# JoeMWatson/input-inference-for-control

Measured on AMD Instinct MI355X. Metric: i2c timestep-messages/sec (cell-iterations/s = B*T*EM-iters/s), pendulum T=200 B=4096 per GPU, higher is better.
Workload: dtype f64; 1 GPU; pendulum_known_quad cubature i2c (nx=2, nu=1, nz=4), T=200, B=4096 trajectories per GPU, global batch 4096, CubatureQuadrature(1,0,0), alpha0=100, tol=0; batch_per_gpu=4096, horizon=200, parallelism=batch-sharded x1, no collective in the EM loop, kernels=one lane per trajectory

## Files before the change

input-inference-for-control_amd/csrc/i2c_cell.hpp:

```cpp
#pragma once
#include <stdint.h>
#include <type_traits>
#include "../../include/i2c_hip.h"
#include "i2c_linalg.hpp"
#include "i2c_models.hpp"

namespace i2c {

template <typename R> struct Rule {
  R sf;
  R w0;
  R wi;
  R W;
  int unit;
  int gh_degree, gh_points;
  R gh_x[I2C_MAX_GH_DEGREE], gh_w[I2C_MAX_GH_DEGREE];
};

template <class M> struct PerTraj : M {};
template <class M> struct is_per_traj : std::false_type {};
template <class M> struct is_per_traj<PerTraj<M>> : std::true_type {};
template <typename R, bool PER_TRAJ> struct ParamsB {};
template <typename R> struct ParamsB<R, true> {
  const R* params_b;
// ... 120 lines not shown
  I2C_HD static constexpr int lin(int) { return -1; }
  I2C_HD static constexpr int dep(int) { return DIN - 1; }
};

template <class M, class ST, int DIN, int DOUT, bool CROSS, bool UNITW = false, typename R, class F>
I2C_FN void sp_transform(const Rule<R>& rule, const R* m, const R* Sin, const R* L, const F& f, R* my, R* Sy,
                         R* Sxy, const PolyTab<R>* tab = nullptr) {
  constexpr int NA = M::NA, NA1 = NA > 0 ? NA : 1;
  R s0[NA1], c0[NA1];
#pragma unroll
  for (int a = 0; a < NA; ++a) {
    if (tab)
      r_sincos(m[M::ang(a)], *tab, &s0[a], &c0[a]);
    else
      r_sincos(m[M::ang(a)], &s0[a], &c0[a]);
  }
  R y0[DOUT];
  f(m, s0, c0, y0);
  R A[DOUT];
#pragma unroll
  for (int k = 0; k < DOUT; ++k) A[k] = R(0);
#pragma unroll
  for (int k = 0; k < sym(DOUT); ++k) Sy[k] = R(0);
  if (CROSS) {
#pragma unroll
    for (int k = 0; k < DIN * DOUT; ++k) Sxy[k] = R(0);
  }
#pragma unroll
  for (int j = 0; j < DIN; ++j) {
    bool any = false;
#pragma unroll
    for (int k = 0; k < DOUT; ++k) any = any || (ST::lin(k) < 0 && ST::dep(k) >= j);
    R a[DOUT], dl[DOUT];
    if (any) {
      R xp[DIN], xm[DIN];
#pragma unroll
      for (int i = 0; i < DIN; ++i) {
        if (i < j) {
          xp[i] = m[i];
          xm[i] = m[i];
        } else {
          const R d = rule.sf * L[tri(i, j)];
          xp[i] = m[i] + d;
          xm[i] = m[i] - d;
        }
      }
      R sp[NA1], cp[NA1], sm[NA1], cm[NA1];
#pragma unroll
      for (int q = 0; q < NA; ++q) {
        if (M::ang(q) < j) {
          sp[q] = sm[q] = s0[q];
          cp[q] = cm[q] = c0[q];
        } else {
          R sd, cd;
          if (tab)
            r_sincos(rule.sf * L[tri(M::ang(q), j)], *tab, &sd, &cd);
          else
            r_sincos_small(rule.sf * L[tri(M::ang(q), j)], &sd, &cd);
          sp[q] = s0[q] * cd + c0[q] * sd;
          cp[q] = c0[q] * cd - s0[q] * sd;
          sm[q] = s0[q] * cd - c0[q] * sd;
          cm[q] = c0[q] * cd + s0[q] * sd;
        }
      }
      R yp[DOUT], ym[DOUT];
      f(xp, sp, cp, yp);
      f(xm, sm, cm, ym);
#pragma unroll
      for (int k = 0; k < DOUT; ++k) {
        a[k] = (yp[k] - y0[k]) + (ym[k] - y0[k]);
        dl[k] = yp[k] - ym[k];
      }
    }
#pragma unroll
    for (int k = 0; k < DOUT; ++k) {
      const bool nl_k = ST::lin(k) < 0 && ST::dep(k) >= j;
      if (ST::lin(k) >= j) dl[k] = R(2) * rule.sf * L[tri(ST::lin(k) >= j ? ST::lin(k) : j, j)];
      if (nl_k) A[k] += a[k];
#pragma unroll
      for (int l = 0; l <= k; ++l) {
        const bool nl_l = ST::lin(l) < 0 && ST::dep(l) >= j;
        const bool d_k = nl_k || ST::lin(k) >= j, d_l = nl_l || ST::lin(l) >= j;
        const bool both_lin = ST::lin(k) >= 0 && ST::lin(l) >= 0;
        if (nl_k && nl_l) Sy[tri(k, l)] += a[k] * a[l];
        if (d_k && d_l && !both_lin) Sy[tri(k, l)] += dl[k] * dl[l];
      }
      if (CROSS && nl_k) {
#pragma unroll
        for (int i = j; i < DIN; ++i) Sxy[i * DOUT + k] += L[tri(i, j)] * dl[k];
      }
    }
    sched_fence<(DIN >= 6)>();
  }
  const R hw = R(0.5) * rule.wi, w2 = rule.wi * rule.wi, cs = rule.wi * rule.sf;
#pragma unroll
  for (int k = 0; k < DOUT; ++k) {
    const R Wk = UNITW ? R(1) : rule.W;
    my[k] = ST::lin(k) >= 0 ? Wk * m[ST::lin(k) >= 0 ? ST::lin(k) : 0] : Wk * y0[k] + rule.wi * A[k];
#pragma unroll
    for (int l = 0; l <= k; ++l) {
      if (ST::lin(k) >= 0 && ST::lin(l) >= 0)
        Sy[tri(k, l)] = Sin[tri_any(ST::lin(k) >= 0 ? ST::lin(k) : 0, ST::lin(l) >= 0 ? ST::lin(l) : 0)];
      else
        Sy[tri(k, l)] = hw * Sy[tri(k, l)] - w2 * A[k] * A[l];
    }
    if (CROSS) {
#pragma unroll
      for (int i = 0; i < DIN; ++i)
        Sxy[i * DOUT + k] = ST::lin(k) >= 0 ? Sin[tri_any(i, ST::lin(k) >= 0 ? ST::lin(k) : 0)] : cs * Sxy[i * DOUT + k];
    }
  }
  if (!UNITW && !rule.unit) {
    const R omw = R(1) - rule.W;
    R yc[DOUT];
#pragma unroll
    for (int k = 0; k < DOUT; ++k) yc[k] = ST::lin(k) >= 0 ? m[ST::lin(k) >= 0 ? ST::lin(k) : 0] : y0[k];
#pragma unroll
    for (int k = 0; k < DOUT; ++k)
#pragma unroll
      for (int l = 0; l <= k; ++l)
        Sy[tri(k, l)] += omw * (rule.W * yc[k] * yc[l] + rule.wi * (A[k] * yc[l] + yc[k] * A[l]));
  }
}

template <int DX, int DZ, typename R>
I2C_FN bool kalman_update(R* mu, R* S, const R* mz, R* Sz, R* Sxz, const R* zt) {
  R rinv[DZ];
  const bool ok = chol<DZ>(Sz, rinv);
  R q[DZ];
#pragma unroll
  for (int k = 0; k < DZ; ++k) q[k] = zt[k] - mz[k];
  fsub<DZ>(Sz, rinv, q);
#pragma unroll
  for (int i = 0; i < DX; ++i) {
    fsub<DZ>(Sz, rinv, &Sxz[i * DZ]);
    R v = mu[i];
#pragma unroll
    for (int k = 0; k < DZ; ++k) v += Sxz[i * DZ + k] * q[k];
    mu[i] = v;
    sched_fence<(DZ >= 8)>();
  }
#pragma unroll
  for (int i = 0; i < DX; ++i)
#pragma unroll
    for (int j = 0; j <= i; ++j) {
      R v = S[tri(i, j)];
#pragma unroll
      for (int k = 0; k < DZ; ++k) v -= Sxz[i * DZ + k] * Sxz[j * DZ + k];
      S[tri(i, j)] = v;
    }
  return ok;
}

template <int N, typename R> I2C_FN R pdf_ratio(R* S, const R* delta, bool* ok, const PolyTab<R>* tab = nullptr) {
  R rinv[N], q[N];
  *ok = chol<N>(S, rinv);
#pragma unroll
  for (int i = 0; i < N; ++i) q[i] = delta[i];
  fsub<N>(S, rinv, q);
  R maha = R(0);
#pragma unroll
  for (int i = 0; i < N; ++i) maha += q[i] * q[i];
  (void)tab;
  return r_exp(R(-0.5) * maha);
}

template <int NX, int NU, typename R>
I2C_FN void joint_from_gain(const R* mu_x, const R* sig_x, const R* Kt, const R* qmu_x, const R* qmu_u,
                            const R* sig_u, R* mu0, R* S0) {
  constexpr int D = NX + NU;
#pragma unroll
  for (int i = 0; i < NX; ++i) mu0[i] = mu_x[i];
#pragma unroll
  for (int a = 0; a < NU; ++a) {
    R v = qmu_u[a];
#pragma unroll
    for (int k = 0; k < NX; ++k) v += Kt[a * NX + k] * (mu_x[k] - qmu_x[k]);
    mu0[NX + a] = v;
  }
#pragma unroll
  for (int i = 0; i < NX; ++i)
#pragma unroll
    for (int j = 0; j <= i; ++j) S0[tri(i, j)] = sig_x[tri(i, j)];
#pragma unroll
  for (int a = 0; a < NU; ++a) {
#pragma unroll
    for (int j = 0; j < NX; ++j) {
      R v = R(0);
#pragma unroll
      for (int k = 0; k < NX; ++k) v += Kt[a * NX + k] * sig_x[tri_any(k, j)];
      S0[tri(NX + a, j)] = v;
    }
#pragma unroll
    for (int c = 0; c <= a; ++c) S0[tri(NX + a, NX + c)] = sig_u[tri(a, c)];
  }
  (void)D;
}

template <int NX, int NU, typename R> I2C_FN void gain_quad(const R* Kt, const R* sig, R* out) {
  R KS[NU * NX];
#pragma unroll
  for (int a = 0; a < NU; ++a)
#pragma unroll
    for (int j = 0; j < NX; ++j) {
      R v = R(0);
#pragma unroll
      for (int k = 0; k < NX; ++k) v += Kt[a * NX + k] * sig[tri_any(k, j)];
      KS[a * NX + j] = v;
    }
#pragma unroll
  for (int a = 0; a < NU; ++a)
#pragma unroll
    for (int c = 0; c <= a; ++c) {
      R v = R(0);
#pragma unroll
      for (int j = 0; j < NX; ++j) v += KS[a * NX + j] * Kt[c * NX + j];
      out[tri(a, c)] = v;
    }
}

I2C_FN int note_failure(int fail, bool ok, int reason, int t) {
  return (fail == 0 && !ok) ? ((reason << 16) | (t + 1)) : fail;
}
I2C_FN int flag_stage(int cell_bad, bool ok, int order) {
  const int v = ok ? 0 : 7 - order;
  return cell_bad > v ? cell_bad : v;
}
I2C_FN int fold_cell_failure(int fail, int cell_bad, int t) {
  const int order = 7 - cell_bad;
  const int reason = order == 0 ? 2 : (order == 1 ? 1 : order + 1);
  return (fail == 0 && cell_bad != 0) ? ((reason << 16) | (t + 1)) : fail;
}
I2C_FN void set_status(int32_t* status, int b, int reason, int t) {
  if (status[b] == 0) status[b] = (reason << 16) | (t + 1);
}

template <class M, int DIN, int DOUT, bool CROSS, typename R, class F>
I2C_FN void grid_transform(const Rule<R>& rule, const R* m, const R* L, const F& f, R* my, R* Sy, R* Sxy) {
  constexpr int NA = M::NA, NA1 = NA > 0 ? NA : 1;
  R sn[NA1], cs[NA1], y0[DOUT], s1[DOUT];
#pragma unroll
  for (int a = 0; a < NA; ++a) r_sincos(m[M::ang(a)], &sn[a], &cs[a]);
  f(m, sn, cs, y0);
#pragma unroll
  for (int k = 0; k < DOUT; ++k) s1[k] = R(0);
#pragma unroll
  for (int k = 0; k < sym(DOUT); ++k) Sy[k] = R(0);
  if (CROSS) {
#pragma unroll
    for (int k = 0; k < DIN * DOUT; ++k) Sxy[k] = R(0);
  }
  int dig[DIN];
#pragma unroll
  for (int i = 0; i < DIN; ++i) dig[i] = 0;
  const int deg = rule.gh_degree;
  for (int p = 0; p < rule.gh_points; ++p) {
    R xi[DIN], w = R(1);
#pragma unroll
    for (int i = 0; i < DIN; ++i) {
      R xv = rule.gh_x[0], wv = rule.gh_w[0];
#pragma unroll
      for (int q = 1; q < I2C_MAX_GH_DEGREE; ++q) {
        xv = dig[i] == q ? rule.gh_x[q] : xv;
        wv = dig[i] == q ? rule.gh_w[q] : wv;
      }
      xi[i] = xv;
      w *= wv;
    }
    R dx[DIN], x[DIN], y[DOUT];
#pragma unroll
    for (int i = 0; i < DIN; ++i) {
      R v = R(0);
#pragma unroll
      for (int j = 0; j <= i; ++j) v += L[tri(i, j)] * xi[j];
      dx[i] = rule.sf * v;
      x[i] = m[i] + dx[i];
    }
#pragma unroll
    for (int a = 0; a < NA; ++a) r_sincos(x[M::ang(a)], &sn[a], &cs[a]);
    f(x, sn, cs, y);
#pragma unroll
    for (int k = 0; k < DOUT; ++k) y[k] -= y0[k];
#pragma unroll
    for (int k = 0; k < DOUT; ++k) {
      const R wy = w * y[k];
      s1[k] += wy;
#pragma unroll
      for (int l = 0; l <= k; ++l) Sy[tri(k, l)] += wy * y[l];
      if (CROSS) {
#pragma unroll
        for (int i = 0; i < DIN; ++i) Sxy[i * DOUT + k] += dx[i] * wy;
      }
    }
    bool carry = true;
#pragma unroll
    for (int i = 0; i < DIN; ++i) {
      const int nd = dig[i] + (carry ? 1 : 0);
      carry = nd >= deg;
      dig[i] = carry ? 0 : nd;
    }
  }
#pragma unroll
  for (int k = 0; k < DOUT; ++k) my[k] = y0[k] + s1[k];
#pragma unroll
  for (int k = 0; k < DOUT; ++k)
#pragma unroll
    for (int l = 0; l <= k; ++l) Sy[tri(k, l)] -= s1[k] * s1[l];
}

template <class M, int DEG, int DIN, int DOUT, bool CROSS, typename R, class F>
I2C_FN void grid_transform_ct(const Rule<R>& rule, const R* m, const R* L, const F& f, R* my, R* Sy, R* Sxy) {
  static_assert(DIN >= 1 && DIN <= 3, "unrolled grid: up to three input dimensions");
  constexpr int NA = M::NA, NA1 = NA > 0 ? NA : 1;
  R sn[NA1], cs[NA1], y0[DOUT], s1[DOUT];
#pragma unroll
  for (int a = 0; a < NA; ++a) r_sincos(m[M::ang(a)], &sn[a], &cs[a]);
  f(m, sn, cs, y0);
#pragma unroll
  for (int k = 0; k < DOUT; ++k) s1[k] = R(0);
#pragma unroll
  for (int k = 0; k < sym(DOUT); ++k) Sy[k] = R(0);
  if (CROSS) {
#pragma unroll
    for (int k = 0; k < DIN * DOUT; ++k) Sxy[k] = R(0);
  }
  R xs[DEG], ws[DEG];
#pragma unroll
  for (int q = 0; q < DEG; ++q) xs[q] = rule.sf * rule.gh_x[q], ws[q] = rule.gh_w[q];
  constexpr int N1 = DIN > 1 ? DEG : 1, N2 = DIN > 2 ? DEG : 1;
#pragma unroll
  for (int i0 = 0; i0 < DEG; ++i0) {
    R d0[DIN];
#pragma unroll
    for (int i = 0; i < DIN; ++i) d0[i] = L[tri(i, 0)] * xs[i0];
#pragma unroll
    for (int a = 0; a < NA; ++a)
      if (M::ang(a) == 0) r_sincos(m[0] + d0[0], &sn[a], &cs[a]);
#pragma unroll
    for (int i1 = 0; i1 < N1; ++i1) {
      R d1[DIN];
      R w1 = ws[i0];
#pragma unroll
      for (int i = 0; i < DIN; ++i) d1[i] = d0[i];
      if constexpr (DIN > 1) {
#pragma unroll
        for (int i = 1; i < DIN; ++i) d1[i] += L[tri(i, 1)] * xs[i1];
        w1 *= ws[i1];
#pragma unroll
        for (int a = 0; a < NA; ++a)
          if (M::ang(a) == 1) r_sincos(m[1] + d1[1], &sn[a], &cs[a]);
      }
      R part[DOUT];
#pragma unroll
      for (int k = 0; k < DOUT; ++k) part[k] = R(0);
#pragma unroll
      for (int i2 = 0; i2 < N2; ++i2) {
        R dx[DIN], x[DIN], y[DOUT];
        R w = w1;
#pragma unroll
        for (int i = 0; i < DIN; ++i) dx[i] = d1[i];
        if constexpr (DIN > 2) {
          dx[2] += L[tri(2, 2)] * xs[i2];
          w *= ws[i2];
#pragma unroll
          for (int a = 0; a < NA; ++a)
            if (M::ang(a) == 2) r_sincos(m[2] + dx[2], &sn[a], &cs[a]);
        }
#pragma unroll
        for (int i = 0; i < DIN; ++i) x[i] = m[i] + dx[i];
        f(x, sn, cs, y);
#pragma unroll
        for (int k = 0; k < DOUT; ++k) {
          const R wy = w * (y[k] - y0[k]);
          y[k] -= y0[k];
          part[k] += wy;
#pragma unroll
          for (int l = 0; l <= k; ++l) Sy[tri(k, l)] += wy * y[l];
          if (CROSS) Sxy[(DIN - 1) * DOUT + k] += dx[DIN - 1] * wy;
        }
      }
#pragma unroll
      for (int k = 0; k < DOUT; ++k) {
        s1[k] += part[k];
        if (CROSS) {
#pragma unroll
          for (int i = 0; i < DIN - 1; ++i) Sxy[i * DOUT + k] += d1[i] * part[k];
        }
      }
    }
  }
#pragma unroll
  for (int k = 0; k < DOUT; ++k) my[k] = y0[k] + s1[k];
#pragma unroll
  for (int k = 0; k < DOUT; ++k)
#pragma unroll
    for (int l = 0; l <= k; ++l) Sy[tri(k, l)] -= s1[k] * s1[l];
}

template <bool GRID, class M, class ST, int DIN, int DOUT, bool CROSS, bool UNITW = false, typename R, class F>
I2C_FN void transform(const Rule<R>& rule, const R* m, const R* Sin, const R* L, const F& f, R* my, R* Sy, R* Sxy,
                      const PolyTab<R>* tab = nullptr) {
  if constexpr (GRID) {
    if constexpr (DIN <= 3) {
      if (rule.gh_degree == 3) return grid_transform_ct<M, 3, DIN, DOUT, CROSS>(rule, m, L, f, my, Sy, Sxy);
      if (rule.gh_degree == 4) return grid_transform_ct<M, 4, DIN, DOUT, CROSS>(rule, m, L, f, my, Sy, Sxy);
      if (rule.gh_degree == 2) return grid_transform_ct<M, 2, DIN, DOUT, CROSS>(rule, m, L, f, my, Sy, Sxy);
    }
    grid_transform<M, DIN, DOUT, CROSS>(rule, m, L, f, my, Sy, Sxy);
  } else
    sp_transform<M, ST, DIN, DOUT, CROSS, UNITW>(rule, m, Sin, L, f, my, Sy, Sxy, tab);
}


template <typename R, typename S = R> struct FwdArgs {
  const S* prior;
  S* fwd;
  S* prior_out;
  const R* x0;
  const R* sig_x0;
  const R* z;
  const R* alpha;
  const R* alpha_cell;
  const uint8_t* ff;
  int32_t* status;
  const uint8_t* expert;
};

template <class M, typename R, bool LEAN = false, bool GRID = false, typename ST_ = R>
I2C_HD inline void forward_sweep_body(const Consts<M, R>& c, const FwdArgs<R, ST_>& a, const int b) {
  using C = Consts<M, R>;
  constexpr int NX = C::NX, NU = C::NU, NZ = C::NZ, NZT = C::NZT, D = C::D;
  constexpr unsigned W = sizeof(ST_);
  const unsigned long B = c.B;
  const int T = c.T;
  const unsigned bo = (unsigned)b * W;
  const unsigned rb0 = (unsigned)(B * W);
  const R alpha_traj = a.alpha[b];
  int fail = 0;

  R mu_x[NX], sig_x[sym(NX)];
#pragma unroll
  for (int i = 0; i < NX; ++i) mu_x[i] = a.x0[i * B + b];
#pragma unroll
  for (int i = 0; i < sym(NX); ++i) sig_x[i] = a.sig_x0[i * B + b];

  constexpr bool VOFF = C::D <= 5;
  unsigned voff[VOFF ? C::E_FWD : 1];
  if (VOFF) {
#pragma unroll
    for (int e = 0; e < C::E_FWD; ++e) voff[e] = bo + (unsigned)e * rb0;
  }
  constexpr bool PREFETCH = C::D <= 5;
  R pri[C::E_PRI], zt[NZ];
  if (PREFETCH) {
    const unsigned rb = rb0;
    const Window w = make_window(a.prior + (unsigned long)(LEAN ? 0 : c.row(0)) * C::E_POST * B, (unsigned long)C::E_POST * rb);
#pragma unroll
    for (int e = 0; e < C::E_PRI; ++e) pri[e] = (R)wld<ST_>(w, VOFF ? 0u : (e) * rb, VOFF ? voff[e] : bo);
#pragma unroll
    for (int k = 0; k < NZ; ++k) zt[k] = (!LEAN && c.z_per_cell) ? a.z[((long)c.row(0) * NZ + k) * B + b] : c.zg[k];
  }

  unsigned ff_cur = a.ff[LEAN ? 0 : c.row(0)];
  constexpr bool STRUCT_L0 = C::D <= 5;
  R Lx[STRUCT_L0 ? sym(NX) : 1];
  if (STRUCT_L0) {
    R rx[NX];
#pragma unroll
    for (int i = 0; i < sym(NX); ++i) Lx[i] = sig_x[i];
    fail = note_failure(fail, chol<NX>(Lx, rx), 1, 0);
  }

  ff_cur = opaque(ff_cur);
  if (PREFETCH) {
#pragma unroll
    for (int e = 0; e < C::E_PRI; ++e) pri[e] = opaque(pri[e]);
#pragma unroll
    for (int k = 0; k < NZ; ++k) zt[k] = opaque(zt[k]);
  }
#pragma unroll
  for (int i = 0; i < NX; ++i) mu_x[i] = opaque(mu_x[i]);
#pragma unroll
  for (int i = 0; i < sym(NX); ++i) sig_x[i] = opaque(sig_x[i]);
  const R alpha_settled = opaque(alpha_traj);
  R alpha_cur = opaque((!LEAN && a.alpha_cell) ? a.alpha_cell[(long)c.row(0) * B + b] : alpha_settled);
  constexpr bool CONST_V = VOFF && (sym(NZ) + sym(NX) <= 16);
  PolyTab<R> ptab;
  if (CONST_V) poly_tab_init(ptab);
  const PolyTab<R>* const tab = CONST_V ? &ptab : nullptr;
  R xi0_v[CONST_V ? sym(NZ) : 1], eta_v[CONST_V ? sym(NX) : 1];
  if (CONST_V) {
#pragma unroll
    for (int i = 0; i < sym(NZ); ++i) xi0_v[i] = opaque(c.sig_xi0[i]);
#pragma unroll
    for (int i = 0; i < sym(NX); ++i) eta_v[i] = opaque(LEAN ? c.sig_eta[i] : c.sig_eta_w[i]);
  }

  for (int t = 0; t < T; ++t) {
    const int tn = t + 1 < T ? t + 1 : t;
    const int tr = LEAN ? t : c.row(t), tnr = LEAN ? tn : c.row(tn);
    const unsigned rb = opaque_uniform(rb0);
    const int kz = (C::D >= 6) ? (int)opaque_uniform(0u) : 0;
    if (!PREFETCH) {
      const Window w = make_window(a.prior + (unsigned long)tr * C::E_POST * B, (unsigned long)C::E_POST * rb);
#pragma unroll
      for (int e = 0; e < C::E_PRI; ++e) pri[e] = (R)wld<ST_>(w, VOFF ? 0u : (e) * rb, VOFF ? voff[e] : bo);
#pragma unroll
      for (int k = 0; k < NZ; ++k) zt[k] = (!LEAN && c.z_per_cell) ? a.z[((long)tr * NZ + k) * B + b] : c.zg[k];
    }

    const R alpha = opaque(alpha_cur);
    const R* pmu = pri;
    const R* psig = pri + D;
    const R* Kprev = pri + D + sym(D);

    int cell_bad = 0;
    R mu0[D], S0[sym(D)];
    R L0[STRUCT_L0 ? sym(D) : 1], Luu[sym(NU)], ruu[NU];
    if (ff_cur != 0) {
#pragma unroll
      for (int i = 0; i < NX; ++i) mu0[i] = mu_x[i];
#pragma unroll
      for (int i = NX; i < D; ++i) mu0[i] = pmu[i];
#pragma unroll
      for (int i = 0; i < D; ++i)
#pragma unroll
        for (int j = 0; j <= i; ++j)
          S0[tri(i, j)] = (i < NX) ? sig_x[tri(i, j)] : (j >= NX ? psig[tri(i, j)] : R(0));
      if (STRUCT_L0) {
#pragma unroll
        for (int p = 0; p < NU; ++p)
#pragma unroll
          for (int q = 0; q <= p; ++q) Luu[tri(p, q)] = psig[tri(NX + p, NX + q)];
#pragma unroll
        for (int p = 0; p < NU; ++p)
#pragma unroll
          for (int j = 0; j < NX; ++j) L0[tri(NX + p, j)] = R(0);
      }
    } else {
      R S[sym(NX)], delta[NX];
#pragma unroll
      for (int i = 0; i < sym(NX); ++i) S[i] = psig[i] + sig_x[i];
#pragma unroll
      for (int i = 0; i < NX; ++i) delta[i] = mu_x[i] - pmu[i];
      bool ok;
      const R rho = pdf_ratio<NX>(S, delta, &ok, tab);
      cell_bad = flag_stage(cell_bad, ok, 0);
      R Kt[NU * NX];
#pragma unroll
      for (int i = 0; i < NU * NX; ++i) Kt[i] = rho * Kprev[i];
      R sig_u[sym(NU)];
      gain_quad<NX, NU>(Kt, sig_x, sig_u);
#pragma unroll
      for (int p = 0; p < NU; ++p)
#pragma unroll
        for (int q = 0; q <= p; ++q) {
          R v = psig[tri(NX + p, NX + q)];
#pragma unroll
          for (int k = 0; k < NX; ++k) v -= Kt[p * NX + k] * psig[tri(NX + q, k)];
          Luu[tri(p, q)] = v;
          sig_u[tri(p, q)] += v;
        }
      joint_from_gain<NX, NU>(mu_x, sig_x, Kt, pmu, pmu + NX, sig_u, mu0, S0);
      if (STRUCT_L0) {
#pragma unroll
        for (int p = 0; p < NU; ++p)
#pragma unroll
          for (int j = 0; j < NX; ++j) {
            R v = R(0);
#pragma unroll
            for (int k = j; k < NX; ++k) v += Kt[p * NX + k] * Lx[tri(k, j)];
            L0[tri(NX + p, j)] = v;
          }
      }
    }
    if (STRUCT_L0) {
#pragma unroll
      for (int i = 0; i < sym(NX); ++i) L0[i] = Lx[i];
      cell_bad = flag_stage(cell_bad, chol<NU>(Luu, ruu), 1);
#pragma unroll
      for (int p = 0; p < NU; ++p)
#pragma unroll
        for (int q = 0; q <= p; ++q) L0[tri(NX + p, NX + q)] = Luu[tri(p, q)];
    }
    if (!LEAN && a.prior_out) {
      const Window w = make_window(a.prior_out + (unsigned long)t * (D + sym(D)) * B, (unsigned long)(D + sym(D)) * rb);
#pragma unroll
      for (int e = 0; e < D; ++e) wst(w, VOFF ? 0u : (e) * rb, VOFF ? voff[e] : bo, (ST_)mu0[e]);
#pragma unroll
      for (int e = 0; e < sym(D); ++e) wst(w, VOFF ? 0u : (D + e) * rb, VOFF ? voff[D + e] : bo, (ST_)S0[e]);
    }

    ff_cur = a.ff[tnr];
    if (!LEAN && a.alpha_cell) alpha_cur = a.alpha_cell[(long)tnr * B + b];
    if (PREFETCH) {
      const Window w = make_window(a.prior + (unsigned long)tnr * C::E_POST * B, (unsigned long)C::E_POST * rb);
#pragma unroll
      for (int e = 0; e < C::E_PRI; ++e) pri[e] = (R)wld<ST_>(w, VOFF ? 0u : (e) * rb, VOFF ? voff[e] : bo);
    }

    sched_fence<(D >= 6)>();
    {
      R Lf[STRUCT_L0 ? 1 : sym(D)], rinv[D];
      if (!STRUCT_L0) {
#pragma unroll
        for (int i = 0; i < sym(D); ++i) Lf[i] = S0[i];
        cell_bad = flag_stage(cell_bad, chol<D>(Lf, rinv), 1);
      }
      const R* L = STRUCT_L0 ? L0 : Lf;
      R mz[NZ], Sz[sym(NZ)], Sxz[D * NZ];
      transform<GRID, M, ObsStruct<M>, D, NZ, true, LEAN>(c.rule_xu, mu0, S0, L, ObserveF<M, R>{params_of(c, b)}, mz, Sz, Sxz, tab);
#pragma unroll
      for (int i = 0; i < sym(NZ); ++i) Sz[i] += alpha * (CONST_V ? xi0_v[i] : c.sig_xi0[i + kz]);
      cell_bad = flag_stage(cell_bad, kalman_update<D, NZ>(mu0, S0, mz, Sz, Sxz, zt), 2);
    }
    if (!LEAN && PREFETCH && c.z_per_cell) {
#pragma unroll
      for (int k = 0; k < NZ; ++k) zt[k] = a.z[((long)tnr * NZ + k) * B + b];
    }
    const Window out = make_window(a.fwd + (unsigned long)t * C::E_FWD * B, (unsigned long)C::E_FWD * rb);
#pragma unroll
    for (int e = 0; e < D; ++e) wst(out, VOFF ? 0u : (e) * rb, VOFF ? voff[e] : bo, (ST_)mu0[e]);
#pragma unroll
    for (int e = 0; e < sym(D); ++e) wst(out, VOFF ? 0u : (D + e) * rb, VOFF ? voff[D + e] : bo, (ST_)S0[e]);

    sched_fence<(D >= 6)>();
    R Sxy[D * NX];
    {
      R L[sym(D)], rinv[D];
#pragma unroll
      for (int i = 0; i < sym(D); ++i) L[i] = S0[i];
      cell_bad = flag_stage(cell_bad, chol<D>(L, rinv), 3);
      transform<GRID, M, DenseStruct<D>, D, NX, true, LEAN>(c.rule_xu, mu0, S0, L, DynamicsF<M, R>{params_of(c, b)}, mu_x, sig_x, Sxy, tab);
    }
#pragma unroll
    for (int i = 0; i < sym(NX); ++i) sig_x[i] += CONST_V ? eta_v[i] : (LEAN ? c.sig_eta[i + kz] : c.sig_eta_w[i + kz]);
    R L3[sym(NX)], rinv3[NX];
#pragma unroll
    for (int i = 0; i < sym(NX); ++i) L3[i] = sig_x[i];
    cell_bad = flag_stage(cell_bad, chol<NX>(L3, rinv3), 4);
    sched_fence<(D >= 6)>();
#pragma unroll
    for (int i = 0; i < D; ++i) {
      fsub<NX>(L3, rinv3, &Sxy[i * NX]);
      bsub<NX>(L3, rinv3, &Sxy[i * NX]);
      sched_fence<(D >= 6)>();
    }

    ff_cur = opaque(ff_cur);
    if (!LEAN) {
      alpha_cur = opaque(alpha_cur);
      if (PREFETCH) {
#pragma unroll
        for (int k = 0; k < NZ; ++k) zt[k] = opaque(zt[k]);
      }
    }
    if (PREFETCH) {
#pragma unroll
      for (int e = 0; e < C::E_PRI; ++e) pri[e] = opaque(pri[e]);
    }
#pragma unroll
    for (int e = 0; e < D * NX; ++e) wst(out, VOFF ? 0u : (D + sym(D) + NX + sym(NX) + e) * rb, VOFF ? voff[D + sym(D) + NX + sym(NX) + e] : bo, (ST_)Sxy[e]);
    sched_fence<(D >= 6)>();

    if (NZT > 0 && t == c.terminal_cell && c.has_Qf) {
      constexpr int NT = C::NZT1;
      R mzt[NT], Szt[sym(NT)], Sxzt[NX * NT];
      transform<GRID, M, TermStruct<M>, NX, NT, true, LEAN>(c.rule_x, mu_x, sig_x, L3, ObserveTermF<M, R>{params_of(c, b)}, mzt, Szt, Sxzt);
#pragma unroll
      for (int i = 0; i < sym(NT); ++i) Szt[i] += alpha * c.sig_xiT0[i];
      cell_bad = flag_stage(cell_bad, kalman_update<NX, NT>(mu_x, sig_x, mzt, Szt, Sxzt, c.zg_term), 5);
      if (STRUCT_L0) {
#pragma unroll
        for (int i = 0; i < sym(NX); ++i) L3[i] = sig_x[i];
        cell_bad = flag_stage(cell_bad, chol<NX>(L3, rinv3), 5);
      }
    }
    if (STRUCT_L0) {
#pragma unroll
      for (int i = 0; i < sym(NX); ++i) Lx[i] = L3[i];
    }
    fail = fold_cell_failure(fail, cell_bad, t);
#pragma unroll
    for (int e = 0; e < NX; ++e) wst(out, VOFF ? 0u : (D + sym(D) + e) * rb, VOFF ? voff[D + sym(D) + e] : bo, (ST_)mu_x[e]);
#pragma unroll
    for (int e = 0; e < sym(NX); ++e) wst(out, VOFF ? 0u : (D + sym(D) + NX + e) * rb, VOFF ? voff[D + sym(D) + NX + e] : bo, (ST_)sig_x[e]);

  }
  if (fail != 0 && a.status[b] == 0) a.status[b] = fail;
}


template <class M, typename R>
I2C_FN void end_of_chain(const Consts<M, R>& c, R* temp, const int b, const R* m3f, const R* S3f, R* m3m, R* S3m,
                         int32_t* status) {
  constexpr int NX = M::NX;
  if (c.has_x_terminal) {
    const R tmp = temp[b];
    temp[b] = tmp + c.dtemp;
    R St[sym(NX)], Ssum[sym(NX)], rinv[NX];
#pragma unroll
    for (int i = 0; i < sym(NX); ++i) {
      St[i] = tmp * S3f[i];
      Ssum[i] = c.sig_x_term[i] + St[i];
    }
    bool ok = chol<NX>(Ssum, rinv);
    R Wm[NX * NX];
#pragma unroll
    for (int j = 0; j < NX; ++j) {
      R col[NX];
#pragma unroll
      for (int i = 0; i < NX; ++i) col[i] = St[tri_any(i, j)];
      fsub<NX>(Ssum, rinv, col);
#pragma unroll
      for (int i = 0; i < NX; ++i) Wm[i * NX + j] = col[i];
    }
#pragma unroll
    for (int i = 0; i < NX; ++i)
#pragma unroll
      for (int j = 0; j <= i; ++j) {
        R v = St[tri(i, j)];
#pragma unroll
        for (int k = 0; k < NX; ++k) v -= Wm[k * NX + i] * Wm[k * NX + j];
        S3m[tri(i, j)] = v;
      }
    R r1[NX], r2[NX], Lt[sym(NX)], LT[sym(NX)];
#pragma unroll
    for (int i = 0; i < sym(NX); ++i) {
      Lt[i] = St[i];
      LT[i] = c.sig_x_term[i];
    }
    ok = chol<NX>(Lt, rinv) && ok;
#pragma unroll
    for (int i = 0; i < NX; ++i) r1[i] = m3f[i];
    fsub<NX>(Lt, rinv, r1);
    bsub<NX>(Lt, rinv, r1);
    ok = chol<NX>(LT, rinv) && ok;
#pragma unroll
    for (int i = 0; i < NX; ++i) r2[i] = c.mu_x_term[i];
    fsub<NX>(LT, rinv, r2);
    bsub<NX>(LT, rinv, r2);
#pragma unroll
    for (int i = 0; i < NX; ++i) r1[i] += r2[i];
    symv<NX>(S3m, r1, m3m);
    if (!ok) set_status(status, b, 6, c.T - 1);
  } else {
#pragma unroll
    for (int i = 0; i < NX; ++i) m3m[i] = m3f[i];
#pragma unroll
    for (int i = 0; i < sym(NX); ++i) S3m[i] = S3f[i];
  }
}

template <int N, typename R>
I2C_FN void gaussian_cost(const R* W, const bool w_diag, const R* mz, const R* Sz, const R* zt, R* m, R* v) {
  R err[N];
#pragma unroll
  for (int i = 0; i < N; ++i) err[i] = mz[i] - zt[i];
  if (w_diag) {
    R mm = R(0), tr2 = R(0), quad = R(0), we[N];
#pragma unroll
    for (int i = 0; i < N; ++i) {
      we[i] = W[tri(i, i)] * err[i];
      mm += we[i] * err[i] + W[tri(i, i)] * Sz[tri(i, i)];
    }
#pragma unroll
    for (int i = 0; i < N; ++i)
#pragma unroll
      for (int j = 0; j <= i; ++j) {
        const R sww = Sz[tri(i, j)] * (W[tri(i, i)] * W[tri(j, j)]);
        tr2 += (i == j ? R(1) : R(2)) * Sz[tri(i, j)] * sww;
        quad += (i == j ? R(1) : R(2)) * Sz[tri(i, j)] * (we[i] * we[j]);
      }
    *m = mm;
    *v = R(2) * tr2 + R(4) * quad;
    return;
  }
  R We[N];
  symv<N>(W, err, We);
  R SW[N * N];
#pragma unroll
  for (int i = 0; i < N; ++i)
#pragma unroll
    for (int j = 0; j < N; ++j) {
      R s = R(0);
#pragma unroll
      for (int k = 0; k < N; ++k) s += Sz[tri_any(i, k)] * W[tri_any(k, j)];
      SW[i * N + j] = s;
    }
  R mm = R(0), tr2 = R(0), quad = R(0);
#pragma unroll
  for (int i = 0; i < N; ++i) {
    mm += err[i] * We[i] + SW[i * N + i];
    R SWe = R(0);
#pragma unroll
    for (int j = 0; j < N; ++j) {
      tr2 += SW[i * N + j] * SW[j * N + i];
      SWe += Sz[tri_any(i, j)] * We[j];
    }
    quad += We[i] * SWe;
  }
  *m = mm;
  *v = R(2) * tr2 + R(4) * quad;
}

template <class M, typename R, bool GRID = false>
I2C_FN R terminal_obs_stats(const Consts<M, R>& c, const int b, const R* m3m, const R* S3m, R* term_stats,
                            int32_t* status) {
  using C = Consts<M, R>;
  constexpr int NX = C::NX, NZT = C::NZT;
  const long B = c.B;
  R trT = R(0);
  if (NZT > 0 && c.has_Qf) {
    constexpr int NT = C::NZT1;
    R L3[sym(NX)], rinv3[NX], mzt[NT], Szt[sym(NT)];
#pragma unroll
    for (int i = 0; i < sym(NX); ++i) L3[i] = S3m[i];
    if (!chol<NX>(L3, rinv3)) set_status(status, b, 6, c.T - 1);
    transform<GRID, M, TermStruct<M>, NX, NT, false>(c.rule_x, m3m, S3m, L3, ObserveTermF<M, R>{params_of(c, b)}, mzt, Szt,
                                                  (R*)nullptr);
    R tv;
    gaussian_cost<NT>(c.Qf, c.qf_diag != 0, mzt, Szt, c.zg_term, &trT, &tv);
#pragma unroll
    for (int k = 0; k < NT; ++k) term_stats[(long)(3 + k) * B + b] = mzt[k];
#pragma unroll
    for (int k = 0; k < sym(NT); ++k) term_stats[(long)(3 + NT + k) * B + b] = Szt[k];
  }
  term_stats[b] = trT;
  return trT;
}

template <class M, typename R, bool GRID = false>
I2C_FN bool cell_posterior(const Consts<M, R>& c, const int b, const R* zt, R* mu, R* S, const R* J, const R* dm, const R* dS,
                           R* ctl, R* mz, R* Sz, R* cm, R* cv, const PolyTab<R>* tab = nullptr) {
  using C = Consts<M, R>;
// ... 972 lines not shown
```

input-inference-for-control_amd/csrc/i2c_linalg.hpp:

```cpp
#pragma once

#ifdef I2C_HOST_SIM
#include <cmath>
#define I2C_HD
#else
#include <hip/hip_runtime.h>
#define I2C_HD __host__ __device__
#endif
#define I2C_FN I2C_HD static inline __attribute__((always_inline))

namespace i2c {

constexpr int sym(int n) { return n * (n + 1) / 2; }
constexpr int tri(int i, int j) { return i * (i + 1) / 2 + j; }
constexpr int tri_any(int i, int j) { return i >= j ? tri(i, j) : tri(j, i); }

#ifdef I2C_HOST_SIM
I2C_FN double seed_rsq(double x) { return (double)(float)(1.0 / std::sqrt(x)); }
I2C_FN double seed_rcp(double x) { return (double)(float)(1.0 / x); }
I2C_FN double m_fma(double a, double b, double c) { return std::fma(a, b, c); }
I2C_FN double m_rint(double x) { return std::rint(x); }
I2C_FN double m_fabs(double x) { return std::fabs(x); }
I2C_FN float r_rsqrt(float x) { return 1.0f / std::sqrt(x); }
I2C_FN float r_rcp(float x) { return 1.0f / x; }
I2C_FN double r_exp(double x) { return std::exp(x); }
I2C_FN float r_exp(float x) { return std::exp(x); }
I2C_FN double r_log(double x) { return std::log(x); }
I2C_FN float r_log(float x) { return std::log(x); }
I2C_FN void r_sincos(float x, float* s, float* c) { *s = std::sin(x); *c = std::cos(x); }
#else
I2C_FN double seed_rsq(double x) { return __builtin_amdgcn_rsq(x); }
I2C_FN double seed_rcp(double x) { return __builtin_amdgcn_rcp(x); }
I2C_FN double m_fma(double a, double b, double c) { return fma(a, b, c); }
I2C_FN double m_rint(double x) { return rint(x); }
I2C_FN double m_fabs(double x) { return fabs(x); }
I2C_FN float r_rsqrt(float x) { return rsqrtf(x); }
I2C_FN float r_rcp(float x) { return 1.0f / x; }
I2C_FN float r_exp(float x) { return expf(x); }
I2C_FN double r_log(double x) { return log(x); }
I2C_FN float r_log(float x) { return logf(x); }
I2C_FN void r_sincos(float x, float* s, float* c) { sincosf(x, s, c); }
#endif

#ifdef I2C_HOST_SIM
I2C_FN double p_fma(double p, double z, double c) { return std::fma(p, z, c); }
#else
I2C_FN double p_fma(double p, double z, double c) {
  double r;
  asm("v_fma_f64 %0, %1, %2, %3" : "=v"(r) : "v"(p), "v"(z), "v"(c));
  return r;
}
#endif

I2C_FN double r_rsqrt(double x) {
  const double y = seed_rsq(x);
  const double e = m_fma(-(x * y), y, 1.0);
  return m_fma(y * e, m_fma(e, 0.375, 0.5), y);
}
I2C_FN double r_rcp(double x) {
  double y = seed_rcp(x);
  y = m_fma(m_fma(-x, y, 1.0), y, y);
  return m_fma(m_fma(-x, y, 1.0), y, y);
}
#ifndef I2C_HOST_SIM
I2C_FN double r_exp(double x) {
  const double n = m_rint(x * 1.44269504088896338700e+00);
  double r = m_fma(-n, 6.93147180369123816490e-01, x);
  r = m_fma(-n, 1.90821492927058770002e-10, r);
  const double z = r * r;
  double e = p_fma(2.08767569878681e-09, z, 2.755731922398589e-07);
  double o = p_fma(1.6059043836821613e-10, z, 2.505210838544172e-08);
  e = p_fma(e, z, 2.48015873015873e-05);
  o = p_fma(o, z, 2.7557319223985893e-06);
  e = p_fma(e, z, 1.388888888888889e-03);
  o = p_fma(o, z, 1.984126984126984e-04);
  e = p_fma(e, z, 4.1666666666666664e-02);
  o = p_fma(o, z, 8.333333333333333e-03);
  e = p_fma(e, z, 0.5);
  o = p_fma(o, z, 1.6666666666666666e-01);
  e = m_fma(e, z, 1.0);
  o = m_fma(o, z, 1.0);
  return __builtin_ldexp(m_fma(r, o, e), (int)n);
}
#endif

I2C_FN void r_sincos(double x, double* s, double* c) {
  x = m_fabs(x) < 1.0e6 ? x : __builtin_nan("");
  const double n = m_rint(x * 6.36619772367581382433e-01);
  double r = m_fma(-n, 1.57079632673412561417e+00, x);
  r = m_fma(-n, 6.07710050630396597660e-11, r);
  r = m_fma(-n, 2.02226624871116645580e-21, r);
  const double z = r * r;
  double ps = p_fma(z, 1.58969099521155010221e-10, -2.50507602534068634195e-08);
  ps = p_fma(ps, z, 2.75573137070700676789e-06);
  ps = p_fma(ps, z, -1.98412698298579493134e-04);
  ps = p_fma(ps, z, 8.33333333332248946124e-03);
  const double sr = m_fma(z * r, m_fma(z, ps, -1.66666666666666324348e-01), r);
  double pc = p_fma(z, -1.13596475577881948265e-11, 2.08757232129817482790e-09);
  pc = p_fma(pc, z, -2.75573143513906633035e-07);
  pc = p_fma(pc, z, 2.48015872894767294178e-05);
  pc = p_fma(pc, z, -1.38888888888741095749e-03);
  pc = p_fma(pc, z, 4.16666666666666019037e-02);
  const double cr = 1.0 - m_fma(0.5, z, -(z * z) * pc);
  const int q = (int)n;
  const double ss = (q & 1) ? cr : sr;
  const double cc = (q & 1) ? sr : cr;
  *s = (q & 2) ? -ss : ss;
  *c = ((q + 1) & 2) ? -cc : cc;
}
#ifdef I2C_HOST_SIM
I2C_FN void r_sincos_sc(double x, double* s, double* c) { r_sincos(x, s, c); }
I2C_FN double r_exp_sc(double x) { return r_exp(x); }
#else
I2C_FN double p_fma_s(double p, double z, double c) {
  double r;
  asm("v_fma_f64 %0, %1, %2, %3" : "=v"(r) : "v"(p), "v"(z), "s"(c));
  return r;
}
I2C_FN void r_sincos_sc(double x, double* s, double* c) {
  x = m_fabs(x) < 1.0e6 ? x : __builtin_nan("");
  const double n = m_rint(x * 6.36619772367581382433e-01);
  double r = m_fma(-n, 1.57079632673412561417e+00, x);
  r = m_fma(-n, 6.07710050630396597660e-11, r);
  r = m_fma(-n, 2.02226624871116645580e-21, r);
  const double z = r * r;
  double ps = p_fma_s(z * 1.58969099521155010221e-10, 1.0, -2.50507602534068634195e-08);
  ps = p_fma_s(ps, z, 2.75573137070700676789e-06);
  ps = p_fma_s(ps, z, -1.98412698298579493134e-04);
  ps = p_fma_s(ps, z, 8.33333333332248946124e-03);
  const double sr = m_fma(z * r, p_fma_s(z, ps, -1.66666666666666324348e-01), r);
  double pc = p_fma_s(z * -1.13596475577881948265e-11, 1.0, 2.08757232129817482790e-09);
  pc = p_fma_s(pc, z, -2.75573143513906633035e-07);
  pc = p_fma_s(pc, z, 2.48015872894767294178e-05);
  pc = p_fma_s(pc, z, -1.38888888888741095749e-03);
  pc = p_fma_s(pc, z, 4.16666666666666019037e-02);
  const double cr = 1.0 - m_fma(0.5, z, -(z * z) * pc);
  const int q = (int)n;
  const double ss = (q & 1) ? cr : sr;
  const double cc = (q & 1) ? sr : cr;
  *s = (q & 2) ? -ss : ss;
  *c = ((q + 1) & 2) ? -cc : cc;
}
I2C_FN double r_exp_sc(double x) {
  const double n = m_rint(x * 1.44269504088896338700e+00);
  double r = m_fma(-n, 6.93147180369123816490e-01, x);
  r = m_fma(-n, 1.90821492927058770002e-10, r);
  const double z = r * r;
  double e = p_fma_s(z * 2.08767569878681e-09, 1.0, 2.755731922398589e-07);
  double o = p_fma_s(z * 1.6059043836821613e-10, 1.0, 2.505210838544172e-08);
  e = p_fma_s(e, z, 2.48015873015873e-05);
  o = p_fma_s(o, z, 2.7557319223985893e-06);
  e = p_fma_s(e, z, 1.388888888888889e-03);
  o = p_fma_s(o, z, 1.984126984126984e-04);
  e = p_fma_s(e, z, 4.1666666666666664e-02);
  o = p_fma_s(o, z, 8.333333333333333e-03);
  e = p_fma_s(e, z, 0.5);
  o = p_fma_s(o, z, 1.6666666666666666e-01);
  e = m_fma(e, z, 1.0);
  o = m_fma(o, z, 1.0);
  return __builtin_ldexp(m_fma(r, o, e), (int)n);
}
#endif

template <typename R> struct PolyTab {
  R two_over_pi, pio2_1, pio2_2, pio2_3, s1, s2, s3, s4, s5, s6, c1, c2, c3, c4, c5, c6;
};
template <typename R> I2C_FN R tab_value(double v) {
  R x = (R)v;
#ifndef I2C_HOST_SIM
  asm volatile("" : "+v"(x));
#endif
  return x;
}
template <typename R> I2C_FN void poly_tab_init(PolyTab<R>& t) {
  t.two_over_pi = tab_value<R>(6.36619772367581382433e-01);
  t.pio2_1 = tab_value<R>(1.57079632673412561417e+00);
  t.pio2_2 = tab_value<R>(6.07710050630396597660e-11);
  t.pio2_3 = tab_value<R>(2.02226624871116645580e-21);
  t.s6 = tab_value<R>(1.58969099521155010221e-10);
  t.s5 = tab_value<R>(-2.50507602534068634195e-08);
  t.s4 = tab_value<R>(2.75573137070700676789e-06);
  t.s3 = tab_value<R>(-1.98412698298579493134e-04);
  t.s2 = tab_value<R>(8.33333333332248946124e-03);
  t.s1 = tab_value<R>(-1.66666666666666324348e-01);
  t.c6 = tab_value<R>(-1.13596475577881948265e-11);
  t.c5 = tab_value<R>(2.08757232129817482790e-09);
  t.c4 = tab_value<R>(-2.75573143513906633035e-07);
  t.c3 = tab_value<R>(2.48015872894767294178e-05);
  t.c2 = tab_value<R>(-1.38888888888741095749e-03);
  t.c1 = tab_value<R>(4.16666666666666019037e-02);
}
I2C_FN void r_sincos(double x, const PolyTab<double>& t, double* s, double* c) {
  x = m_fabs(x) < 1.0e6 ? x : __builtin_nan("");
  const double n = m_rint(x * t.two_over_pi);
  double r = m_fma(-n, t.pio2_1, x);
  r = m_fma(-n, t.pio2_2, r);
  r = m_fma(-n, t.pio2_3, r);
  const double z = r * r;
  double ps = p_fma(z, t.s6, t.s5);
  ps = p_fma(ps, z, t.s4);
  ps = p_fma(ps, z, t.s3);
  ps = p_fma(ps, z, t.s2);
  const double sr = m_fma(z * r, p_fma(z, ps, t.s1), r);
  double pc = p_fma(z, t.c6, t.c5);
  pc = p_fma(pc, z, t.c4);
  pc = p_fma(pc, z, t.c3);
  pc = p_fma(pc, z, t.c2);
  pc = p_fma(pc, z, t.c1);
  const double cr = 1.0 - m_fma(0.5, z, -(z * z) * pc);
  const int q = (int)n;
  const double ss = (q & 1) ? cr : sr;
  const double cc = (q & 1) ? sr : cr;
  *s = (q & 2) ? -ss : ss;
  *c = ((q + 1) & 2) ? -cc : cc;
}
I2C_FN void r_sincos(float x, const PolyTab<float>&, float* s, float* c) { r_sincos(x, s, c); }

I2C_FN void r_sincos_small(double x, double* s, double* c) { r_sincos(x, s, c); }
I2C_FN void r_sincos_small(float x, float* s, float* c) { r_sincos(x, s, c); }

#ifdef I2C_HOST_SIM
struct Window {
  char* p;
};
I2C_FN Window make_window(const void* base, unsigned long) { return Window{(char*)base}; }
template <typename R> I2C_FN R wld(const Window& w, unsigned row_off, unsigned lane_off) {
  return *reinterpret_cast<const R*>(w.p + row_off + lane_off);
}
template <typename R> I2C_FN void wst(const Window& w, unsigned row_off, unsigned lane_off, R v) {
  *reinterpret_cast<R*>(w.p + row_off + lane_off) = v;
}
I2C_FN unsigned wld_u8(const Window& w, unsigned off) { return *reinterpret_cast<const unsigned char*>(w.p + off); }
template <typename S> struct Pair2 {
  S a, b;
};
template <typename S> I2C_FN Pair2<S> wld2(const Window& w, unsigned row_off, unsigned lane_off) {
  const S* q = reinterpret_cast<const S*>(w.p + row_off + lane_off);
  return Pair2<S>{q[0], q[1]};
}
template <typename S> I2C_FN void wst2(const Window& w, unsigned row_off, unsigned lane_off, Pair2<S> v) {
  S* q = reinterpret_cast<S*>(w.p + row_off + lane_off);
  q[0] = v.a, q[1] = v.b;
}
#else
struct Window {
  __amdgpu_buffer_rsrc_t r;
};
I2C_FN unsigned uniform_u32(unsigned x) { return (unsigned)__builtin_amdgcn_readfirstlane((int)x); }
I2C_FN Window make_window(const void* base, unsigned long bytes) {
  const unsigned long p = (unsigned long)base;
  const unsigned long pu = ((unsigned long)uniform_u32((unsigned)(p >> 32)) << 32) | uniform_u32((unsigned)p);
  const unsigned n = uniform_u32(bytes > 0xFFFFFFFFul ? 0xFFFFFFFFu : (unsigned)bytes);
  return Window{__builtin_amdgcn_make_buffer_rsrc((void*)pu, 0, n, 0x00020000)};
}
template <typename R> I2C_FN R wld(const Window& w, unsigned row_off, unsigned lane_off) {
  if constexpr (sizeof(R) == 8) {
    typedef unsigned v2u __attribute__((ext_vector_type(2)));
    const v2u v = __builtin_amdgcn_raw_buffer_load_b64(w.r, lane_off, uniform_u32(row_off), 0);
    return __builtin_bit_cast(R, v);
  } else {
    return __builtin_bit_cast(R, __builtin_amdgcn_raw_buffer_load_b32(w.r, lane_off, uniform_u32(row_off), 0));
  }
}
I2C_FN unsigned wld_u8(const Window& w, unsigned off) { return (unsigned)__builtin_amdgcn_raw_buffer_load_b8(w.r, off, 0, 0); }
I2C_FN void wst(const Window& w, unsigned row_off, unsigned lane_off, double v) {
  typedef unsigned v2u __attribute__((ext_vector_type(2)));
  __builtin_amdgcn_raw_buffer_store_b64(__builtin_bit_cast(v2u, v), w.r, lane_off, uniform_u32(row_off), 0);
}
I2C_FN void wst(const Window& w, unsigned row_off, unsigned lane_off, float v) {
  __builtin_amdgcn_raw_buffer_store_b32(__builtin_bit_cast(unsigned, v), w.r, lane_off, uniform_u32(row_off), 0);
}
template <typename S> struct Pair2 {
  S a, b;
};
template <typename S> I2C_FN Pair2<S> wld2(const Window& w, unsigned row_off, unsigned lane_off) {
  if constexpr (sizeof(S) == 8) {
    typedef unsigned v4u __attribute__((ext_vector_type(4)));
    const v4u v = __builtin_amdgcn_raw_buffer_load_b128(w.r, lane_off, uniform_u32(row_off), 0);
    return __builtin_bit_cast(Pair2<S>, v);
  } else {
    typedef unsigned v2u __attribute__((ext_vector_type(2)));
    const v2u v = __builtin_amdgcn_raw_buffer_load_b64(w.r, lane_off, uniform_u32(row_off), 0);
    return __builtin_bit_cast(Pair2<S>, v);
  }
}
template <typename S> I2C_FN void wst2(const Window& w, unsigned row_off, unsigned lane_off, Pair2<S> v) {
  if constexpr (sizeof(S) == 8) {
    typedef unsigned v4u __attribute__((ext_vector_type(4)));
    __builtin_amdgcn_raw_buffer_store_b128(__builtin_bit_cast(v4u, v), w.r, lane_off, uniform_u32(row_off), 0);
  } else {
    typedef unsigned v2u __attribute__((ext_vector_type(2)));
    __builtin_amdgcn_raw_buffer_store_b64(__builtin_bit_cast(v2u, v), w.r, lane_off, uniform_u32(row_off), 0);
  }
}
#endif

template <bool ON> I2C_FN void sched_fence() {
#ifndef I2C_HOST_SIM
  if (ON) __builtin_amdgcn_sched_barrier(0);
#endif
}

I2C_FN unsigned opaque_uniform(unsigned x) {
#ifndef I2C_HOST_SIM
  asm volatile("" : "+s"(x));
#endif
  return x;
}
template <typename R> I2C_FN R opaque(R x) {
#ifndef I2C_HOST_SIM
  asm volatile("" : "+v"(x));
#endif
  return x;
}

#ifdef I2C_HOST_SIM
template <typename R> I2C_FN R r_clip(R x, R lo, R hi) { return x < lo ? lo : (x > hi ? hi : x); }
#else
I2C_FN double r_clip(double x, double lo, double hi) { return fmin(fmax(x, lo), hi); }
I2C_FN float r_clip(float x, float lo, float hi) { return fminf(fmaxf(x, lo), hi); }
#endif

template <int N, typename R> I2C_FN bool chol(R* a, R* rinv) {
  bool ok = true;
#pragma unroll
  for (int j = 0; j < N; ++j) {
    R s = a[tri(j, j)];
#pragma unroll
    for (int k = 0; k < j; ++k) s -= a[tri(j, k)] * a[tri(j, k)];
    if (j == N - 1) ok = s > R(0);
    const R r = r_rsqrt(s);
    rinv[j] = r;
    a[tri(j, j)] = s * r;
#pragma unroll
    for (int i = j + 1; i < N; ++i) {
      R v = a[tri(i, j)];
#pragma unroll
      for (int k = 0; k < j; ++k) v -= a[tri(i, k)] * a[tri(j, k)];
      a[tri(i, j)] = v * r;
    }
  }
  return ok;
}

template <int N, typename R> I2C_FN bool chol_signed(R* a, R* rinv, R* sgn) {
  bool ok = true;
#pragma unroll
  for (int j = 0; j < N; ++j) {
    R s = a[tri(j, j)];
#pragma unroll
    for (int k = 0; k < j; ++k) s -= sgn[k] * a[tri(j, k)] * a[tri(j, k)];
    const R g = s < R(0) ? R(-1) : R(1);
    sgn[j] = g;
    s *= g;
    if (j == N - 1) ok = s > R(0);
    const R r = r_rsqrt(s);
    rinv[j] = r;
    a[tri(j, j)] = s * r;
#pragma unroll
    for (int i = j + 1; i < N; ++i) {
      R v = a[tri(i, j)];
#pragma unroll
      for (int k = 0; k < j; ++k) v -= sgn[k] * a[tri(i, k)] * a[tri(j, k)];
      a[tri(i, j)] = v * r * g;
    }
  }
  return ok;
}

// ... 54 lines not shown
```

Measured before the change: 2.343 billion timestep-messages/s.

## Streamline per-cell failure tracking, sign flips, and exp constants in i2c cell

Replaces the running max-based failure code with per-stage boolean flags, folded only when a wave-wide ballot shows any lane failed. It also makes the feed-forward branch condition wave-uniform via readfirstlane, and replaces the sincos sign selects with XOR bit flips. It adds an ExpTab that keeps exp range-reduction constants in registers for the pdf ratio when constant-variance mode is active. Together these aim to cut per-cell VALU and select instructions and SGPR/literal pressure in the inner timestep loop. The readfirstlane assumes ff_cur is uniform across the wave, and the extra register-resident constants may raise register pressure.

New measurement: 2.366 billion timestep-messages/s, median of 6. About the same (+1.0%).

```diff
diff --git a/input-inference-for-control_amd/csrc/i2c_cell.hpp b/input-inference-for-control_amd/csrc/i2c_cell.hpp
--- a/input-inference-for-control_amd/csrc/i2c_cell.hpp
+++ b/input-inference-for-control_amd/csrc/i2c_cell.hpp
@@ -296,7 +296,8 @@
   return ok;
 }
 
-template <int N, typename R> I2C_FN R pdf_ratio(R* S, const R* delta, bool* ok, const PolyTab<R>* tab = nullptr) {
+template <int N, typename R> I2C_FN R pdf_ratio(R* S, const R* delta, bool* ok, const PolyTab<R>* tab = nullptr,
+                                                const ExpTab<R>* etab = nullptr) {
   R rinv[N], q[N];
   *ok = chol<N>(S, rinv);
 #pragma unroll
@@ -306,7 +307,7 @@
 #pragma unroll
   for (int i = 0; i < N; ++i) maha += q[i] * q[i];
   (void)tab;
-  return r_exp(R(-0.5) * maha);
+  return etab ? r_exp(R(-0.5) * maha, *etab) : r_exp(R(-0.5) * maha);
 }
 
 template <int NX, int NU, typename R>
@@ -374,6 +375,28 @@
   const int order = 7 - cell_bad;
   const int reason = order == 0 ? 2 : (order == 1 ? 1 : order + 1);
   return (fail == 0 && cell_bad != 0) ? ((reason << 16) | (t + 1)) : fail;
+}
+struct CellOk {
+  bool pdf = true, prior = true, obs = true, upd = true, pred = true, term = true;
+};
+I2C_FN bool any_lane(bool x) {
+#ifdef I2C_HOST_SIM
+  return x;
+#else
+  return __builtin_amdgcn_ballot_w64(x) != 0;
+#endif
+}
+I2C_FN int fold_cell_ok(int fail, const CellOk& k, int t) {
+  const int reason = !k.pdf ? 2 : !k.prior ? 1 : !k.obs ? 3 : !k.upd ? 4 : !k.pred ? 5 : 6;
+  const bool bad = !(k.pdf && k.prior && k.obs && k.upd && k.pred && k.term);
+  return (fail == 0 && bad) ? ((reason << 16) | (t + 1)) : fail;
+}
+I2C_FN unsigned uniform_flag(unsigned x) {
+#ifdef I2C_HOST_SIM
+  return x;
+#else
+  return (unsigned)__builtin_amdgcn_readfirstlane((int)x);
+#endif
 }
 I2C_FN void set_status(int32_t* status, int b, int reason, int t) {
   if (status[b] == 0) status[b] = (reason << 16) | (t + 1);
@@ -632,6 +655,9 @@
   PolyTab<R> ptab;
   if (CONST_V) poly_tab_init(ptab);
   const PolyTab<R>* const tab = CONST_V ? &ptab : nullptr;
+  ExpTab<R> etab_v;
+  if (CONST_V) exp_tab_init(etab_v);
+  const ExpTab<R>* const etab = CONST_V ? &etab_v : nullptr;
   R xi0_v[CONST_V ? sym(NZ) : 1], eta_v[CONST_V ? sym(NX) : 1];
   if (CONST_V) {
 #pragma unroll
@@ -658,10 +684,10 @@
     const R* psig = pri + D;
     const R* Kprev = pri + D + sym(D);
 
-    int cell_bad = 0;
+    CellOk ok_;
     R mu0[D], S0[sym(D)];
     R L0[STRUCT_L0 ? sym(D) : 1], Luu[sym(NU)], ruu[NU];
-    if (ff_cur != 0) {
+    if (uniform_flag(ff_cur) != 0) {
 #pragma unroll
       for (int i = 0; i < NX; ++i) mu0[i] = mu_x[i];
 #pragma unroll
@@ -687,9 +713,7 @@
       for (int i = 0; i < sym(NX); ++i) S[i] = psig[i] + sig_x[i];
 #pragma unroll
       for (int i = 0; i < NX; ++i) delta[i] = mu_x[i] - pmu[i];
-      bool ok;
-      const R rho = pdf_ratio<NX>(S, delta, &ok, tab);
-      cell_bad = flag_stage(cell_bad, ok, 0);
+      const R rho = pdf_ratio<NX>(S, delta, &ok_.pdf, tab, etab);
       R Kt[NU * NX];
 #pragma unroll
       for (int i = 0; i < NU * NX; ++i) Kt[i] = rho * Kprev[i];
@@ -721,7 +745,7 @@
     if (STRUCT_L0) {
 #pragma unroll
       for (int i = 0; i < sym(NX); ++i) L0[i] = Lx[i];
-      cell_bad = flag_stage(cell_bad, chol<NU>(Luu, ruu), 1);
+      ok_.prior = chol<NU>(Luu, ruu);
 #pragma unroll
       for (int p = 0; p < NU; ++p)
 #pragma unroll
@@ -749,14 +773,14 @@
       if (!STRUCT_L0) {
 #pragma unroll
         for (int i = 0; i < sym(D); ++i) Lf[i] = S0[i];
-        cell_bad = flag_stage(cell_bad, chol<D>(Lf, rinv), 1);
+        ok_.prior = chol<D>(Lf, rinv);
       }
       const R* L = STRUCT_L0 ? L0 : Lf;
       R mz[NZ], Sz[sym(NZ)], Sxz[D * NZ];
       transform<GRID, M, ObsStruct<M>, D, NZ, true, LEAN>(c.rule_xu, mu0, S0, L, ObserveF<M, R>{params_of(c, b)}, mz, Sz, Sxz, tab);
 #pragma unroll
       for (int i = 0; i < sym(NZ); ++i) Sz[i] += alpha * (CONST_V ? xi0_v[i] : c.sig_xi0[i + kz]);
-      cell_bad = flag_stage(cell_bad, kalman_update<D, NZ>(mu0, S0, mz, Sz, Sxz, zt), 2);
+      ok_.obs = kalman_update<D, NZ>(mu0, S0, mz, Sz, Sxz, zt);
     }
     if (!LEAN && PREFETCH && c.z_per_cell) {
 #pragma unroll
@@ -774,7 +798,7 @@
       R L[sym(D)], rinv[D];
 #pragma unroll
       for (int i = 0; i < sym(D); ++i) L[i] = S0[i];
-      cell_bad = flag_stage(cell_bad, chol<D>(L, rinv), 3);
+      ok_.upd = chol<D>(L, rinv);
       transform<GRID, M, DenseStruct<D>, D, NX, true, LEAN>(c.rule_xu, mu0, S0, L, DynamicsF<M, R>{params_of(c, b)}, mu_x, sig_x, Sxy, tab);
     }
 #pragma unroll
@@ -782,7 +806,7 @@
     R L3[sym(NX)], rinv3[NX];
 #pragma unroll
     for (int i = 0; i < sym(NX); ++i) L3[i] = sig_x[i];
-    cell_bad = flag_stage(cell_bad, chol<NX>(L3, rinv3), 4);
+    ok_.pred = chol<NX>(L3, rinv3);
     sched_fence<(D >= 6)>();
 #pragma unroll
     for (int i = 0; i < D; ++i) {
@@ -813,18 +837,18 @@
       transform<GRID, M, TermStruct<M>, NX, NT, true, LEAN>(c.rule_x, mu_x, sig_x, L3, ObserveTermF<M, R>{params_of(c, b)}, mzt, Szt, Sxzt);
 #pragma unroll
       for (int i = 0; i < sym(NT); ++i) Szt[i] += alpha * c.sig_xiT0[i];
-      cell_bad = flag_stage(cell_bad, kalman_update<NX, NT>(mu_x, sig_x, mzt, Szt, Sxzt, c.zg_term), 5);
+      ok_.term = kalman_update<NX, NT>(mu_x, sig_x, mzt, Szt, Sxzt, c.zg_term);
       if (STRUCT_L0) {
 #pragma unroll
         for (int i = 0; i < sym(NX); ++i) L3[i] = sig_x[i];
-        cell_bad = flag_stage(cell_bad, chol<NX>(L3, rinv3), 5);
+        ok_.term = chol<NX>(L3, rinv3) && ok_.term;
       }
     }
     if (STRUCT_L0) {
 #pragma unroll
       for (int i = 0; i < sym(NX); ++i) Lx[i] = L3[i];
     }
-    fail = fold_cell_failure(fail, cell_bad, t);
+    if (any_lane(!(ok_.pdf && ok_.prior && ok_.obs && ok_.upd && ok_.pred && ok_.term))) fail = fold_cell_ok(fail, ok_, t);
 #pragma unroll
     for (int e = 0; e < NX; ++e) wst(out, VOFF ? 0u : (D + sym(D) + e) * rb, VOFF ? voff[D + sym(D) + e] : bo, (ST_)mu_x[e]);
 #pragma unroll
diff --git a/input-inference-for-control_amd/csrc/i2c_linalg.hpp b/input-inference-for-control_amd/csrc/i2c_linalg.hpp
--- a/input-inference-for-control_amd/csrc/i2c_linalg.hpp
+++ b/input-inference-for-control_amd/csrc/i2c_linalg.hpp
@@ -84,6 +84,9 @@
 }
 #endif
 
+I2C_FN double flip_sign_if(double x, unsigned m) {
+  return __builtin_bit_cast(double, __builtin_bit_cast(unsigned long long, x) ^ ((unsigned long long)(m & 0x80000000u) << 32));
+}
 I2C_FN void r_sincos(double x, double* s, double* c) {
   x = m_fabs(x) < 1.0e6 ? x : __builtin_nan("");
   const double n = m_rint(x * 6.36619772367581382433e-01);
@@ -105,8 +108,8 @@
   const int q = (int)n;
   const double ss = (q & 1) ? cr : sr;
   const double cc = (q & 1) ? sr : cr;
-  *s = (q & 2) ? -ss : ss;
-  *c = ((q + 1) & 2) ? -cc : cc;
+  *s = flip_sign_if(ss, (unsigned)q << 30);
+  *c = flip_sign_if(cc, (unsigned)(q + 1) << 30);
 }
 #ifdef I2C_HOST_SIM
 I2C_FN void r_sincos_sc(double x, double* s, double* c) { r_sincos(x, s, c); }
@@ -138,8 +141,8 @@
   const int q = (int)n;
   const double ss = (q & 1) ? cr : sr;
   const double cc = (q & 1) ? sr : cr;
-  *s = (q & 2) ? -ss : ss;
-  *c = ((q + 1) & 2) ? -cc : cc;
+  *s = flip_sign_if(ss, (unsigned)q << 30);
+  *c = flip_sign_if(cc, (unsigned)(q + 1) << 30);
 }
 I2C_FN double r_exp_sc(double x) {
   const double n = m_rint(x * 1.44269504088896338700e+00);
@@ -211,10 +214,42 @@
   const int q = (int)n;
   const double ss = (q & 1) ? cr : sr;
   const double cc = (q & 1) ? sr : cr;
-  *s = (q & 2) ? -ss : ss;
-  *c = ((q + 1) & 2) ? -cc : cc;
+  *s = flip_sign_if(ss, (unsigned)q << 30);
+  *c = flip_sign_if(cc, (unsigned)(q + 1) << 30);
 }
 I2C_FN void r_sincos(float x, const PolyTab<float>&, float* s, float* c) { r_sincos(x, s, c); }
+template <typename R> struct ExpTab {
+  R log2e, ln2_hi, ln2_lo;
+};
+template <typename R> I2C_FN void exp_tab_init(ExpTab<R>& t) {
+  t.log2e = tab_value<R>(1.44269504088896338700e+00);
+  t.ln2_hi = tab_value<R>(6.93147180369123816490e-01);
+  t.ln2_lo = tab_value<R>(1.90821492927058770002e-10);
+}
+#ifndef I2C_HOST_SIM
+I2C_FN double r_exp(double x, const ExpTab<double>& t) {
+  const double n = m_rint(x * t.log2e);
+  double r = m_fma(-n, t.ln2_hi, x);
+  r = m_fma(-n, t.ln2_lo, r);
+  const double z = r * r;
+  double e = p_fma(2.08767569878681e-09, z, 2.755731922398589e-07);
+  double o = p_fma(1.6059043836821613e-10, z, 2.505210838544172e-08);
+  e = p_fma(e, z, 2.48015873015873e-05);
+  o = p_fma(o, z, 2.7557319223985893e-06);
+  e = p_fma(e, z, 1.388888888888889e-03);
+  o = p_fma(o, z, 1.984126984126984e-04);
+  e = p_fma(e, z, 4.1666666666666664e-02);
+  o = p_fma(o, z, 8.333333333333333e-03);
+  e = p_fma(e, z, 0.5);
+  o = p_fma(o, z, 1.6666666666666666e-01);
+  e = m_fma(e, z, 1.0);
+  o = m_fma(o, z, 1.0);
+  return __builtin_ldexp(m_fma(r, o, e), (int)n);
+}
+#else
+I2C_FN double r_exp(double x, const ExpTab<double>&) { return r_exp(x); }
+#endif
+I2C_FN float r_exp(float x, const ExpTab<float>&) { return r_exp(x); }
 
 I2C_FN void r_sincos_small(double x, double* s, double* c) { r_sincos(x, s, c); }
 I2C_FN void r_sincos_small(float x, float* s, float* c) { r_sincos(x, s, c); }
```
